# peterdavidfagan/mujoco_robot_environments

Hardware: AMD Instinct MI355X
Metric: env steps/sec (whole node), RearrangementEnv batch=4096 at 1/2/4/8 MI355X (higher is better)
Workload: dtype f32

## Files before the change

### mujoco_robot_environments_amd/csrc/mre_env.h

```cpp
#pragma once
#include <hip/hip_runtime.h>

#include <string>
#include <utility>
#include <vector>

#include "../../include/mre.h"
#include "mre_dev.h"
#include "mre_host.h"
#include "mre_policy.h"

struct mre_env {
  int N = 0, device = 0;
  hipStream_t stream = nullptr;
  mre::DevModel* dM = nullptr;
  mre::DevModel hM;
  int solver = MRE_SOLVER_PGS;
  float *qpos = nullptr, *qvel = nullptr, *qacc_ws = nullptr, *ctrl = nullptr;
  float* qfine = nullptr;
  int *nstep = nullptr, *sv_nstep = nullptr;
  int* nprops = nullptr;
  float* prop_size = nullptr;
  float* osc_target = nullptr;
  uint8_t* grip_closed = nullptr;
// ... 23 lines not shown
  std::vector<std::pair<hipEvent_t, hipEvent_t>> events;
  size_t events_used = 0;
  bool fallback = true;
  unsigned base_flags = 0;
  bool large_only = false;
  bool compact_only = false;
  hipStream_t stream2 = nullptr;
  hipEvent_t ev_fork = nullptr, ev_join = nullptr, ev_order = nullptr;
  uint8_t *d_large = nullptr, *mask_r = nullptr;
  float *sv_qpos = nullptr, *sv_qvel = nullptr, *sv_qacc_ws = nullptr, *sv_ctrl = nullptr, *sv_qfine = nullptr;
  uint32_t* sv_status = nullptr;
  uint8_t* sv_converged = nullptr;
  float* contacts = nullptr;
  float* contacts_full = nullptr;
  int* settle_steps = nullptr;
  int* h_launch_info = nullptr;
  int* d_launch_info = nullptr;
  int* h_info_last = nullptr;
  uint8_t* d_pending = nullptr;
  uint8_t* h_large_stage = nullptr;
  uint8_t* d_large_stage = nullptr;
  bool d_large_stale = false;
  std::vector<uint8_t> h_large, h_rerun;
  int n_large = 0;
  long long* d_env_ids = nullptr;
  int *ps_attempts = nullptr, *ps_prop = nullptr, *ps_tick = nullptr, *ps_which = nullptr;
  double *ps_bounds = nullptr, *ps_pose = nullptr, *ps_zones = nullptr, *ps_pick = nullptr;
  int last_settle_max = 0;
  long long n_reruns = 0, n_promotions = 0, n_demotions = 0;
  struct Group {
    int lo = 0, n = 0;
    hipStream_t st = nullptr, st2 = nullptr;
    hipEvent_t ev_fork = nullptr, ev_join = nullptr;
    struct Out {
      mre::StepArgs args;
      hipEvent_t ev_info = nullptr;
      int stage = 0;
    } out[mre::policy::RING];
    int head = 0, nout = 0;
    int cur = 0;
    int* h_order = nullptr;
    int* d_order = nullptr;
  };
  std::vector<Group> groups;
  int* h_grp_order = nullptr;
  int* d_grp_order = nullptr;
  Group qgroup;
  bool queue_ok = true;
  int queue_ticks = 200;
  int queue_waves = 0;
  int queue_shards = 16;
  int queue_lshards = 8;
  bool queue_test_serial = false;
  int queue_spare_large = 8;
  int queue_run_ticks = 100;
  int queue_min_ticks = 32;
  float tick_tail = 0.f;
  bool tick_tail_valid = false;
  float queue_tail_min = 1.45f;
  unsigned tail_samples = 0;
  std::vector<int> tail_scratch;
  int queue_large_waves_max = 0;
  int* h_qlist = nullptr;
  int* q_ws = nullptr;
  int* q_gen = nullptr;
  int* h_q_err = nullptr;
  int* h_qgrp_order = nullptr;
  long n_queue_launches = 0;
  long long n_handovers = 0;
  int queue_last_handovers = 0;
  static constexpr int RING = mre::policy::RING;
  int ring = 2;
  static constexpr int NSTAGE = mre::policy::NSTAGE;
  hipEvent_t ev_main = nullptr;
  float* seq_copy[RING + 1] = {nullptr, nullptr, nullptr, nullptr, nullptr};
  size_t seq_cap = 0;
  unsigned seq_calls = 0;
  double dbg_wait_s = 0, dbg_call_s = 0; long dbg_calls = 0;
  int calls_since_drain = 0, sync_streak = 0;
  bool broken = false;
};

namespace mre {
int sched_create(mre_env* e);
void sched_destroy(mre_env* e);
int launch_step(mre_env* e, const StepArgs& a, bool settle = false, bool pipeline_ok = true, bool allow_queue = false);
int drain(mre_env* e, bool api_call = false);
}
#define DRAIN(e) do { int rc_ = mre::drain(e, true); if (rc_) return rc_; } while (0)
#define DRAIN_PENDING(e) do { int rc_ = mre::drain(e, false); if (rc_) return rc_; } while (0)

inline int profile_events(mre_env* e, hipEvent_t* e0, hipEvent_t* e1) {
  *e0 = *e1 = nullptr;
  if (!e->profiling) return MRE_OK;
  if (e->events_used == e->events.size()) {
    hipEvent_t x, y;
    HIPCHK(hipEventCreate(&x)); HIPCHK(hipEventCreate(&y));
    e->events.emplace_back(x, y);
  }
  *e0 = e->events[e->events_used].first; *e1 = e->events[e->events_used].second;
  e->events_used++;
  return MRE_OK;
}
```

### mujoco_robot_environments_amd/csrc/mre_kernels.hip

```cpp
#include <hip/hip_runtime.h>

#include "mre_dev.h"
#include "mre_math.h"
#include "mre_collide.h"

namespace mre {
using ModelP = MRE_MODEL_PTR(DevModel);
#if defined(MRE_PHASE_STAMPS) && MRE_PHASE_STAMPS >= 4
__shared__ unsigned long long dbg_acc[4];
#endif

struct OscSm {
  float J[6][7], M[7][7], MiJt[7][6], Li[6][6], Lam[6][6], V[6][6], Jbar[7][6];
  float ep[3], eo[3], F[6], LF[6], tn[7], Jbt[6], xd[6], w[6];
};

struct alignas(8) Blk {
  uint16_t row0;
  uint8_t type, nrows;
  uint8_t rslot;
  uint8_t pa, pb;
  uint8_t primary : 4;
  uint8_t bslot : 4;
};
// ... 1004 lines not shown
      f = (float)(fd - (double)s.qfrc_bias[l]);
    }
    const bool act = prop_is_active(s, dof_pid);
    f = act ? (b < NRB ? f : f - s.qfrc_bias[l]) : 0.f;
    s.qfrc_smooth[l] = f;
    s.qacc_smooth[l] = f;
  }
  MRE_SYNC();
  return arm_mask | (clamped ? 1u << (NU - 1) : 0u);
}
MRE_DEV unsigned smooth_forces(ModelP M, Sm& s, int l) {
  const unsigned arm_mask = arm_actuation(M, s, l);
  const unsigned mask = smooth_forces_assemble(M, s, l, arm_mask);
#ifndef MRE_NEWTON
  solve_robot_one(s.qLD, s.qLDinv, s.qacc_smooth, l);
#else
  factor_solve_robot(s.qM, s.qacc_smooth, l);
#endif
  if (l >= NRV && l < NV) {
    const int p = (l - NRV) / 6, k = (l - NRV) % 6;
    const float md = (k < 3) ? s.prop_mass[p] : s.prop_inertia[p][k - 3];
    s.qacc_smooth[l] = s.qacc_smooth[l] / md;
  }
  MRE_SYNC();
  return mask;
}

MRE_PHASE_FN void integrate_setup(ModelP M, Sm& s, int l, unsigned act_clamped) {
  const bool grip_clamped = (act_clamped >> (NU - 1)) & 1u;
  const float h = M->opt_rec.timestep, grip_bias2 = M->opt_rec.grip_biasprm[2];
  for (int e = l; e < NMR; e += 64) {
    const auto* R = &M->m_rec[e];
    const int i = R->i, j = R->j, ten = R->ten;
    const float damping = R->damping, act_bias2 = R->act_bias2, ten_coef = R->ten_coef;
    float v = s.qM[e];
    if (i == j) {
      v += h * damping;
      if (i < 7 && ((act_clamped >> i) & 1u) == 0u) v -= h * act_bias2;
      if (!grip_clamped) {
        if (ten >= 0) v -= h * grip_bias2 * ten_coef * ten_coef;
      }
    }
    mh_store(s)[e] = v;
#ifdef MRE_NEWTON
    if (i == j) s.scratch[i] = (s.qM[e] - v) * s.qacc[i];
#endif
  }
#ifndef MRE_NEWTON
  if (l < NRV) s.scratch[l] = s.qfrc_smooth[l] + s.qfrc_con[l];
#endif
  MRE_SYNC();
}

MRE_PHASE_FN void integrate(ModelP M, Sm& s, int l, unsigned flags, bool polished, float* clo) {
  const float h = M->opt_rec.timestep;
  const auto* DR = &M->dof_rec[l < NV ? l : 0];
  const int dof_b = DR->body, dof_pid = DR->propid;
  const auto* BR = &M->body_rec[l < NB ? l : 0];
  const int body_qa = BR->qposadr, body_da = BR->dofadr, body_pid = BR->propid;
  const bool freeze = (flags & F_FREEZE_ROBOT) != 0;
  float vl_in = 0.f, ql_in[7] = {0.f, 0.f, 0.f, 0.f, 0.f, 0.f, 0.f};
  if (clo != nullptr) {
    if (l >= NRV && l < NV) vl_in = clo[(QFINE_CUBE_V - QFINE_CUBE_Q) + (l - NRV)];
    if (l >= NRB && l < NB) {
#pragma unroll
      for (int k = 0; k < 7; k++) ql_in[k] = clo[7 * (l - NRB) + k];
    }
  }
  keep_live(dof_pid); keep_live(body_pid); keep_live(body_qa); keep_live(body_da);
  if (l < NV) {
    const int b = dof_b;
    if (b < NRB) {
      if (!freeze) {
#ifdef MRE_NEWTON
        const double acc = polished ? reinterpret_cast<const double*>(&s.nw_Mv[0])[l] : (double)s.qacc[l];
        const double v = robot_v(s, l) + (double)h * (acc + (double)s.scratch[l]);
#else
        const double v = robot_v(s, l) + (double)h * (double)s.scratch[l];
#endif
        const float hi = (float)v;
        s.qvel[l] = hi; s.qlo[QFINE / 2 + l] = (float)(v - (double)hi);
      }
    } else if (prop_is_active(s, dof_pid)) {
      if (clo != nullptr) {
        float* const vl = clo + (QFINE_CUBE_V - QFINE_CUBE_Q) + (l - NRV);
        const double v = (double)s.qvel[l] + (double)vl_in + (double)h * (double)s.qacc[l];
        const float hi = (float)v, lo = (float)(v - (double)hi);
        s.qvel[l] = hi; *vl = lo;
        s.scratch[l] = lo;
      } else {
        s.qvel[l] += h * s.qacc[l];
      }
    }
  }
  MRE_SYNC();
  if (l >= 1 && l < NB) {
    const int b = l, qa = body_qa, da = body_da;
    if (b < NRB) {
      if (!freeze) {
        const double q = robot_q(s, qa) + (double)h * robot_v(s, da);
        const float hi = (float)q;
        s.qpos[qa] = hi; s.qlo[qa] = (float)(q - (double)hi);
      }
    } else if (prop_is_active(s, body_pid) && clo != nullptr) {
      float* const ql = clo + 7 * (b - NRB);
      double vv[6];
      for (int k = 0; k < 6; k++) vv[k] = (double)s.qvel[da + k] + (double)s.scratch[da + k];
      for (int k = 0; k < 3; k++) {
        const double x = (double)s.qpos[qa + k] + (double)ql_in[k] + (double)h * vv[k];
        const float hi = (float)x;
        s.qpos[qa + k] = hi; ql[k] = (float)(x - (double)hi);
      }
      double q0[4], qn[4];
      for (int k = 0; k < 4; k++) q0[k] = (double)s.qpos[qa + 3 + k] + (double)ql_in[3 + k];
      const double wn2 = vv[3] * vv[3] + vv[4] * vv[4] + vv[5] * vv[5];
      if (wn2 > 1e-60) {
        const double inv = rsq64(wn2), half = 0.5 * (double)h * wn2 * inv;
        double sn, cs;
        sincos_poly_d(half, sn, cs);
        const double ax = vv[3] * inv * sn, ay = vv[4] * inv * sn, az = vv[5] * inv * sn;
        qn[0] = q0[0] * cs - q0[1] * ax - q0[2] * ay - q0[3] * az;
        qn[1] = q0[0] * ax + q0[1] * cs + q0[2] * az - q0[3] * ay;
        qn[2] = q0[0] * ay - q0[1] * az + q0[2] * cs + q0[3] * ax;
        qn[3] = q0[0] * az + q0[1] * ay - q0[2] * ax + q0[3] * cs;
      } else {
        for (int k = 0; k < 4; k++) qn[k] = q0[k];
      }
      const double nn = qn[0] * qn[0] + qn[1] * qn[1] + qn[2] * qn[2] + qn[3] * qn[3];
      const double sc = nn > 1e-30 ? rsq64(nn) : 1.0;
      for (int k = 0; k < 4; k++) {
        const double x = qn[k] * sc;
        const float hi = (float)x;
        s.qpos[qa + 3 + k] = hi; ql[3 + k] = (float)(x - (double)hi);
      }
    } else if (prop_is_active(s, body_pid)) {
      for (int k = 0; k < 3; k++) s.qpos[qa + k] += h * s.qvel[da + k];
      float w[3] = {s.qvel[da + 3], s.qvel[da + 4], s.qvel[da + 5]};
      const float ang = v3normalize(w) * h;
      float qr[4], qn[4], q0[4];
      axisangle2q(qr, w, ang);
      for (int k = 0; k < 4; k++) q0[k] = s.qpos[qa + 3 + k];
      qmul(qn, q0, qr);
      qnormalize(qn);
      for (int k = 0; k < 4; k++) s.qpos[qa + 3 + k] = qn[k];
    }
  }
  MRE_SYNC();
}

#ifdef MRE_PHASE_STAMPS
#define MRE_STAMP(k)                                                         \
  do {                                                                       \
    if ((k) < 12 || MRE_PHASE_STAMPS == 3) {                                 \
      const unsigned long long now_ = __builtin_amdgcn_s_memtime();          \
      if ((k) / 4 == MRE_PHASE_STAMPS) stamp_acc[(k) % 4] += now_ - stamp_t; \
      stamp_t = now_;                                                        \
    }                                                                        \
  } while (0)
#else
#define MRE_STAMP(k) do {} while (0)
#endif

MRE_DEV int q_load(const int* p) { return __hip_atomic_load(p, __ATOMIC_RELAXED, __HIP_MEMORY_SCOPE_AGENT); }

#ifdef MRE_LARGE_CAPS
constexpr bool Q_LARGE = true;
#else
constexpr bool Q_LARGE = false;
#endif
MRE_DEV int* q_bucket(const StepArgs& a, int t, int sh) {
  const int S = a.q_shards;
  return a.q_buf + (size_t)t * a.q_stride + (sh < S ? (size_t)sh * a.q_cap : (size_t)S * a.q_cap + (size_t)(sh - S) * a.q_capl);
}

MRE_DEV int queue_pop_shard(const StepArgs& a, int l, int sh, int& env, int& tick) {
  const int S = a.q_shards;
  const bool order0 = sh < S;
  const int n0 = (a.N - sh + S - 1) / S;
  int* const head = a.q_head + sh * QUEUE_TICKS_MAX;
  const int* const tail = a.q_tail + sh * QUEUE_TICKS_MAX;
  for (;;) {
    int h[QUEUE_TICKS_MAX / 64], tl[QUEUE_TICKS_MAX / 64];
#pragma unroll
    for (int c = 0; c < QUEUE_TICKS_MAX / 64; c++) {
      const int b = c * 64 + l;
      h[c] = 0; tl[c] = 0;
      if (b < a.q_nticks) { h[c] = q_load(head + b); tl[c] = (b == 0 && order0) ? n0 : q_load(tail + b); }
    }
    int t = -1, ht = 0;
#pragma unroll
    for (int c = 0; c < QUEUE_TICKS_MAX / 64; c++) {
      if (t < 0 && c * 64 < a.q_nticks) {
        const unsigned long long ready = __ballot(h[c] < tl[c]);
        if (ready != 0ull) {
          const int k = __ffsll((long long)ready) - 1;
          t = c * 64 + k;
          ht = __builtin_amdgcn_readlane(h[c], k);
        }
      }
    }
    if (t < 0) return 0;
    int got = -1;
    if (l == 0) {
      if (t == 0 && order0) {
        const int i = __hip_atomic_fetch_add(head, 1, __ATOMIC_RELAXED, __HIP_MEMORY_SCOPE_AGENT);
        if (i < n0) got = a.env_order != nullptr ? a.env_order[sh + S * i] : sh + S * i;
      } else {
        int expect = ht;
        if (__hip_atomic_compare_exchange_strong(head + t, &expect, ht + 1, __ATOMIC_RELAXED, __ATOMIC_RELAXED,
                                                 __HIP_MEMORY_SCOPE_AGENT)) {
          const int* slot = q_bucket(a, t, sh) + ht;
          int v = q_load(slot);
          for (unsigned spin = 0; v == 0; ++spin) {
            if (spin > (1u << 20)) { *a.q_err = 1; v = -1; break; }
            __builtin_amdgcn_s_sleep(4);
            v = q_load(slot);
          }
          got = v < 0 ? -2 : v - 1;
        }
      }
    }
    got = __builtin_amdgcn_readfirstlane(got);
    if (got == -2) return -1;
    if (got < 0) continue;
    env = got; tick = t;
    return 1;
  }
}
MRE_DEV bool queue_pop(const StepArgs& a, int l, int home, int& env, int& tick, int& shard) {
  const int S = a.q_shards;
  if (Q_LARGE) {
    const int SL = a.q_lshards;
    for (unsigned idle = 0;; ++idle) {
      int r = 0;
      for (int k = 0; k < SL && r == 0; ++k) {
        const int sh = S + (home + k < SL ? home + k : home + k - SL);
        r = queue_pop_shard(a, l, sh, env, tick);
        if (r != 0) shard = sh;
      }
      if (r != 0) return r > 0;
      if (a.q_wait == 0 || q_load(a.q_done) >= a.N) return false;
      if (idle > 512u && q_load(a.q_started) == 0) return false;
      if (idle > (1u << 18)) return false;
      __builtin_amdgcn_s_sleep(127);
    }
  }
  for (int k = 0; k < S; ++k) {
    const int sh = home + k < S ? home + k : home + k - S;
    const int r = queue_pop_shard(a, l, sh, env, tick);
    if (r != 0) { shard = sh; return r > 0; }
  }
  return false;
}
MRE_DEV void queue_push(const StepArgs& a, int l, int env, int tick, int shard) {
  __builtin_amdgcn_fence(__ATOMIC_RELEASE, "agent");
  asm volatile("s_waitcnt vmcnt(0)" ::: "memory");
  if (l == 0) {
    const int i = __hip_atomic_fetch_add(a.q_tail + shard * QUEUE_TICKS_MAX + tick, 1, __ATOMIC_RELAXED, __HIP_MEMORY_SCOPE_AGENT);
    __hip_atomic_store(q_bucket(a, tick, shard) + i, env + 1, __ATOMIC_RELAXED, __HIP_MEMORY_SCOPE_AGENT);
  }
}

template <bool QUEUE>
MRE_DEV void step_body(const StepArgs& a, Sm& s) {
  OscSm& osc = s.osc;
  const int l = threadIdx.x;
  int env = 0, qtick = 0, qshard = 0;
  if (!QUEUE) {
    if ((int)blockIdx.x >= a.N) return;
    env = a.env_order != nullptr ? a.env_order[blockIdx.x] : (int)blockIdx.x;
  }
  if (QUEUE && !Q_LARGE && l == 0) __hip_atomic_fetch_add(a.q_started, 1, __ATOMIC_RELAXED, __HIP_MEMORY_SCOPE_AGENT);
  if (QUEUE && Q_LARGE && a.q_wait != 0) {
    for (unsigned idle = 0; q_load(a.q_gen) != a.q_gen_expect; ++idle) {
      if (idle > 1024u) return;
      __builtin_amdgcn_s_sleep(127);
    }
  }
 for (;;) {
  if (QUEUE) {
    if (!queue_pop(a, l, (int)(blockIdx.x % (unsigned)(Q_LARGE ? a.q_lshards : a.q_shards)), env, qtick, qshard)) return;
    if (qtick > 0 || Q_LARGE) __builtin_amdgcn_fence(__ATOMIC_ACQUIRE, "agent");
  }
  const int step_lo = QUEUE ? qtick * a.control_steps : 0, step_hi = QUEUE ? step_lo + a.control_steps : a.nsteps;
  if (QUEUE && !Q_LARGE && qtick == 0 && a.large != nullptr && a.large[env] != 0) continue;
  if (!QUEUE || (!Q_LARGE && qtick == 0)) {
#define MRE_PASS_SKIP { if (QUEUE) { if (l == 0) __hip_atomic_fetch_add(a.q_done, 1, __ATOMIC_RELAXED, __HIP_MEMORY_SCOPE_AGENT); continue; } return; }
  if (!QUEUE && a.large != nullptr && (a.large[env] != 0) != (a.want_large != 0)) return;
  if (a.env_mask != nullptr && a.env_mask[env] == 0) {
    if (a.launch_info != nullptr && l < 4) a.launch_info[(size_t)env * 4 + l] = -1;
    MRE_PASS_SKIP;
  }
  if (a.pending != nullptr && a.pending[env] != 0) {
    if (a.launch_info != nullptr && l < 4) a.launch_info[(size_t)env * 4 + l] = l == 0 ? -2 : -1;
    MRE_PASS_SKIP;
  }
#undef MRE_PASS_SKIP
  }
  ModelP M = (ModelP)a.M;

  const bool save = a.sv_qpos != nullptr && step_lo == 0;
  if (l < NQP) {
    const float v = a.qpos[(size_t)env * NQP + l];
    s.qpos[l] = v;
    if (save) a.sv_qpos[(size_t)env * NQP + l] = v;
  }
  if (l < NVP) {
    const float v = a.qvel[(size_t)env * NVP + l], w = a.qacc_ws[(size_t)env * NVP + l];
    s.qvel[l] = v;
    s.qacc[l] = w;
    s.qfrc_con[l] = 0.f;
    if (save) { a.sv_qvel[(size_t)env * NVP + l] = v; a.sv_qacc_ws[(size_t)env * NVP + l] = w; }
  }
  if (l < QFINE) {
    const float v = a.qfine != nullptr ? a.qfine[(size_t)env * QFINE_ROW + l] : 0.f;
    s.qlo[l] = v;
    if (save && a.qfine != nullptr) a.sv_qfine[(size_t)env * QFINE_ROW + l] = v;
  }
  if (save && a.qfine != nullptr && l < QFINE_ROW - QFINE)
    a.sv_qfine[(size_t)env * QFINE_ROW + QFINE + l] = a.qfine[(size_t)env * QFINE_ROW + QFINE + l];
  float cube_lo_keep = 0.f;
  if (QUEUE && !Q_LARGE && a.qfine != nullptr && l < QFINE_ROW - QFINE) cube_lo_keep = a.qfine[(size_t)env * QFINE_ROW + QFINE + l];
  if (l < NU) {
    const float v = a.ctrl[(size_t)env * NU + l];
    s.ctrl[l] = v;
    if (save) a.sv_ctrl[(size_t)env * NU + l] = v;
  }
  if (save && l == 0) {
    if (a.nstep != nullptr) a.sv_nstep[env] = a.nstep[env];
    a.sv_status[env] = a.status[env];
    a.sv_converged[env] = a.converged != nullptr ? a.converged[env] : (uint8_t)0;
  }
  if (l == 0) { s.nprops = a.nprops[env]; s.overflow = 0; s.ncon = 0; s.nefc = 0; s.solver_iters = 0; }
#ifdef MRE_NEWTON
  if (l < 24) s.zrow[l] = 0.f;
#endif
  if (l < NPROP * 3) {
    const float sz = a.prop_size[(size_t)env * NPROP * 3 + l];
    s.prop_size[l / 3][l % 3] = sz;
  }
  MRE_SYNC();
  if (l < NPROP) {
    const float m = M->body_mass[NRB + l];
    const float* z = s.prop_size[l];
    s.prop_mass[l] = m;
    s.prop_inertia[l][0] = m / 3.f * (z[1] * z[1] + z[2] * z[2]);
    s.prop_inertia[l][1] = m / 3.f * (z[0] * z[0] + z[2] * z[2]);
    s.prop_inertia[l][2] = m / 3.f * (z[0] * z[0] + z[1] * z[1]);
  }
  MRE_SYNC();

#if defined(MRE_PHASE_STAMPS) && MRE_PHASE_STAMPS >= 4
  if (l < 4) dbg_acc[l] = 0ull;
#endif
#ifdef MRE_PHASE_STAMPS
  unsigned long long stamp_acc[4] = {0, 0, 0, 0};
  unsigned long long stamp_t = __builtin_amdgcn_s_memtime();
#endif
  bool arm_converged = ((a.flags & F_CONV_CONTINUE) != 0 || (QUEUE && qtick > 0)) && a.converged != nullptr && a.converged[env] != 0;
  float grip_cmd = 0.f;
  const OscConfig* oscp = a.osc + (size_t)env * a.osc_stride;
  int hw_ncon = 0, hw_nefc = 0, hw_nrrow = 0, hw_npp = 0;
  const unsigned long long launch_t0 = __builtin_amdgcn_s_memtime();
  if (a.mode == CTRL_OSC) {
    if (l < 16) s.osc_tgt[l] = a.osc_target[(size_t)env * 16 + l];
    grip_cmd = a.grip_closed[env] ? M->act_ctrlrange[NU - 1][1] : M->act_ctrlrange[NU - 1][0];
    MRE_SYNC();
  }
  int steps_done = 0;
  bool settled = false;
  for (int step = step_lo; step < step_hi; ++step) {
    MRE_STAMP(7);
    position_stage(M, s, l);
    MRE_STAMP(12);
    MRE_STAMP(13);
    gripper_local(M, s, l);
    if ((a.flags & F_NO_CONSTRAINTS) == 0) connect_rows_local(M, s, l);
    MRE_STAMP(14);
    crb_mass_matrix(M, s, l);
    MRE_SYNC();
#ifndef MRE_NEWTON
    factor_robot_regs(s.qM, s.qLD, s.qLDinv);
#endif
    MRE_STAMP(15);
    MRE_STAMP(0);

    velocity_stage(M, s, l);
    MRE_SYNC();
    finger_bias(M, s, l);
    MRE_STAMP(1);
    const bool constrained = (a.flags & F_NO_CONSTRAINTS) == 0;
    if (constrained) {

      collide(M, s, l, false, (a.flags & F_CLIP_ALWAYS) != 0);
      MRE_STAMP(2);
      assemble_constraints(M, s, l);
#ifdef MRE_NEWTON
      nw_build_lists(s, l, a.flags);
#else
      solve_robot_rows(s, l);
      assemble_blocks(M, s, l);
#endif
      MRE_STAMP(3);
      hw_ncon = max(hw_ncon, s.ncon); hw_nefc = max(hw_nefc, s.nefc);
      hw_nrrow = max(hw_nrrow, s.nrrow); hw_npp = max(hw_npp, s.npp);
    }

    if (a.mode == CTRL_SEQ && (step % a.control_steps) == 0) {
      const int tick = step / a.control_steps;
      if (l < NU) s.ctrl[l] = a.ctrl_seq[((size_t)tick * a.seq_stride + env) * NU + l];
      MRE_SYNC();
    }
    if (a.mode == CTRL_OSC && (step % a.control_steps) == 0) {
      if (step > 0 && osc_converged(M, s, oscp, s.osc_tgt)) arm_converged = true;
      osc_compute(M, s, osc, oscp, s.osc_tgt, l);
      if (l == 0) s.ctrl[NU - 1] = grip_cmd;
      MRE_SYNC();
    }
    MRE_STAMP(4);
    const unsigned clamped = smooth_forces(M, s, l);
    MRE_STAMP(5);
    bool polished = false;
    if (constrained) {
#if defined(MRE_NEWTON) && defined(MRE_PHASE_STAMPS)
      newton_solve(M, s, l, stamp_acc, stamp_t);
      polished = nw_robot_polish(M, s, l);
#elif defined(MRE_NEWTON)
      newton_solve(M, s, l);
      polished = nw_robot_polish(M, s, l);
#else
      if (M->opt_rec.cone == 0) solve_constraints_pyramidal(M, s, l);
      else solve_constraints(M, s, l);
#endif
      MRE_STAMP(6);
    } else {
      if (l < NVP) { s.qacc[l] = s.qacc_smooth[l]; s.qfrc_con[l] = 0.f; }
      MRE_SYNC();
    }

    integrate_setup(M, s, l, clamped);
    factor_solve_robot(mh_store(s), s.scratch, l);
    integrate(M, s, l, a.flags, polished, a.qfine != nullptr ? a.qfine + (size_t)env * QFINE_ROW + QFINE_CUBE_Q : nullptr);
    steps_done = step + 1 - step_lo;
    if ((a.flags & F_SETTLE_EXIT) != 0) {
      float mv = 0.f, ma = 0.f;
      if (l >= NRV && l < NRV + 6 * s.nprops) { mv = fabsf(s.qvel[l]); ma = fabsf(s.qacc[l]); }
      mv = wave_max(mv); ma = wave_max(ma);
      settled = mv < 1e-3f && ma < 1e-2f && step + 1 > a.min_settle_steps;
    }
    if (a.trace != nullptr && env < a.trace_nenv && (a.trace_base + step) < a.trace_max) {
      if (l < TRACE_QVEL) {
        float v = l < NQ ? s.qpos[l] : 0.f;
        if (l == NQ && constrained) {
          int mask = 0;
          for (int k = 0; k < s.nl; k++) mask |= 1 << ((s.lim_info[k] & 0xFF) - 1);
          v = (float)(s.ncon + 64 * mask);
        }
        if (l == NQ + 1 && constrained) {
          unsigned h = 0u;
          for (int c = 0; c < s.ncon; c++) {
            const int pr = s.con_pair[c];
            const unsigned key = (unsigned)(M->pair_g1[pr] * 32 + M->pair_g2[pr] + 1);
            h = (h + key * key) & 0x3FFFFFu;
          }
          v = (float)h;
        }
        if (l == NQ + 2 && constrained && M->opt_rec.cone != 0) {
          unsigned h = 0u;
          const int ns = 7 + s.nl;
          for (int i = 7; i < ns; i++) h += (s.frc[i] > 0.f ? 1u : 2u) * (unsigned)((i + 1) * (i + 1));
          for (int c = 0; c < s.ncon; c++) {
            const int i = ns + 3 * c;
#ifdef MRE_NEWTON
            const float mu = s.con_fric[c];
#else
            const float mu = s.blkrec[8 + c][15];
#endif
            const float fn = s.frc[i], ft2 = s.frc[i + 1] * s.frc[i + 1] + s.frc[i + 2] * s.frc[i + 2], lim = mu * fn;
            const unsigned z = fn <= 0.f ? 1u : (ft2 >= lim * lim * (1.f - 1e-4f) ? 3u : 2u);
            h += z * (unsigned)((c + 3) * (c + 3));
          }
          v = (float)(h & 0x3FFFFFu);
        }
        a.trace[((size_t)(a.trace_base + step) * a.trace_nenv + env) * TRACE_W + l] = v;
      }
      if (l < NVP) a.trace[((size_t)(a.trace_base + step) * a.trace_nenv + env) * TRACE_W + TRACE_QVEL + l] = l < NV ? s.qvel[l] : 0.f;
    }
    if (settled) break;
  }
  MRE_STAMP(7);
  if (a.settle_steps != nullptr && l == 0) a.settle_steps[env] = settled ? steps_done : -steps_done;
  const bool hand_over = QUEUE && !Q_LARGE && s.overflow != 0;
  if (a.nstep != nullptr && l == 0 && !hand_over) {
    if (QUEUE) __hip_atomic_fetch_add(a.nstep + env, steps_done, __ATOMIC_RELAXED, __HIP_MEMORY_SCOPE_AGENT);
    else a.nstep[env] += steps_done;
  }
  if (a.nsteps == 0 && (a.flags & F_OSC_EVAL) != 0 && a.mode == CTRL_OSC) {
    position_stage(M, s, l);
    gripper_local(M, s, l);
    crb_mass_matrix(M, s, l);
    MRE_SYNC();
    velocity_stage(M, s, l);
    MRE_SYNC();
    osc_compute(M, s, osc, oscp, s.osc_tgt, l);
    if (l == 0) s.ctrl[NU - 1] = grip_cmd;
    MRE_SYNC();
  }
  if (a.nsteps == 0 && (a.flags & F_DETECT) != 0 && a.contacts != nullptr) {
    position_stage(M, s, l);
    collide(M, s, l, (a.flags & F_DETECT_ACTIVE) == 0, (a.flags & F_CLIP_ALWAYS) != 0);
    float* o = a.contacts + (size_t)env * (1 + 3 * CONTACT_EXPORT);
    const int n = s.ncon < CONTACT_EXPORT ? s.ncon : CONTACT_EXPORT;
    if (l == 0) o[0] = s.overflow ? -(float)s.ncon : (float)s.ncon;
    if (l < n) {
      const int pr = s.con_pair[l];
      o[1 + 3 * l] = (float)M->pair_g1[pr]; o[2 + 3 * l] = (float)M->pair_g2[pr]; o[3 + 3 * l] = s.con_dist[l];
      if (a.contacts_full != nullptr) {
        float* f = a.contacts_full + ((size_t)env * CONTACT_EXPORT + l) * 12;
        for (int k = 0; k < 3; k++) f[k] = s.con_pos[l][k];
        for (int k = 0; k < 9; k++) f[3 + k] = s.con_frame[l][k];
      }
    }
    MRE_SYNC();
    if (l == 0) s.overflow = 0;
  }
  const bool q_last = !QUEUE || (qtick + 1 == a.q_nticks && !hand_over);
  if (q_last && (a.mode == CTRL_OSC || a.sites != nullptr || a.geoms != nullptr)) kinematics_only(M, s, l);
  if (a.mode == CTRL_OSC && a.nsteps > 0 && !hand_over) {
    if (q_last && osc_converged(M, s, oscp, s.osc_tgt)) arm_converged = true;
    if (l == 0) {
      if (a.converged != nullptr) a.converged[env] = arm_converged ? 1 : 0;
      if (q_last && !arm_converged && a.status != nullptr && (a.flags & F_CONV_OPEN) == 0) {
        if (QUEUE) __hip_atomic_fetch_or(a.status + env, 1u, __ATOMIC_RELAXED, __HIP_MEMORY_SCOPE_AGENT);
        else a.status[env] |= 1u;
      }
    }
  }
  if (a.geoms != nullptr && l < NG) {
    float p[3], R[9], size[3], rb;
    geom_pose(M, s, l, p, R, size, &rb);
    float* o = a.geoms + ((size_t)env * NG + l) * 16;
    const int pid = M->geom_propid[l];
    const bool active = pid < 0 || pid < s.nprops;
    for (int k = 0; k < 3; k++) o[k] = p[k];
    for (int k = 0; k < 9; k++) o[3 + k] = R[k];
    for (int k = 0; k < 3; k++) o[12 + k] = size[k];
    o[15] = active ? (float)M->geom_type[l] : -1.f;
  }
  if (a.sites != nullptr && q_last) {
    float* o = a.sites + (size_t)env * 16;
    if (l < 3) o[l] = s.site_xpos[M->opt_rec.tcp_site][l];
    if (l >= 3 && l < 6) o[l] = s.site_xpos[M->opt_rec.eef_site][l - 3];
    if (l == 6) {
      float q[4];
      mat2q(q, s.site_xmat[0]);
      o[6] = q[0]; o[7] = q[1]; o[8] = q[2]; o[9] = q[3];
    }
  }
  if (hand_over) {
    if (a.qfine != nullptr && l < QFINE_ROW - QFINE) a.qfine[(size_t)env * QFINE_ROW + QFINE + l] = cube_lo_keep;
  } else {
    if (l < NQP) a.qpos[(size_t)env * NQP + l] = s.qpos[l];
    if (l < NVP) {
      a.qvel[(size_t)env * NVP + l] = s.qvel[l];
      a.qacc_ws[(size_t)env * NVP + l] = l < NV ? s.qacc[l] : 0.f;
    }
    if (l < QFINE && a.qfine != nullptr) a.qfine[(size_t)env * QFINE_ROW + l] = s.qlo[l];
    if (l < NU) a.ctrl[(size_t)env * NU + l] = s.ctrl[l];
  }
  const bool q_more = QUEUE && !hand_over && qtick + 1 < a.q_nticks;
  if (l == 0 && a.launch_info != nullptr) {
    int* li = a.launch_info + (size_t)env * 4;
    unsigned long long dt = (__builtin_amdgcn_s_memtime() - launch_t0) >> 10;
    int moved = 0;
    if (QUEUE) {
      int* qa = a.q_acc + (size_t)env * 4;
      if (qtick > 0 || Q_LARGE) {
        hw_ncon = max(hw_ncon, q_load(qa + 0) & 0xFFFF); hw_nefc = max(hw_nefc, q_load(qa + 1));
        hw_nrrow = max(hw_nrrow, q_load(qa + 2) & 0xFFFF); hw_npp = max(hw_npp, q_load(qa + 2) >> 16);
        dt += (unsigned long long)q_load(qa + 3);
        moved = q_load(qa + 0) >> 16;
      }
      if (hand_over) moved = 1;
      if (q_more || hand_over) { qa[0] = hw_ncon | (moved << 16); qa[1] = hw_nefc; qa[2] = hw_nrrow | (hw_npp << 16); qa[3] = (int)dt; }
      else dt /= (unsigned long long)(qtick + 1);
    }
    if (!q_more && !hand_over) {
#ifdef MRE_LARGE_CAPS
      li[0] = (s.overflow ? 2 : 0) | (moved ? 4 : 0);
#else
      li[0] = s.overflow ? 1 : 0;
#endif
      li[1] = hw_ncon | ((int)(dt < 0x7FFFull ? dt : 0x7FFFull) << 16); li[2] = hw_nefc; li[3] = hw_nrrow | (hw_npp << 16);
    }
  }
#ifndef MRE_LARGE_CAPS
  if (!QUEUE && l == 0 && a.pending != nullptr && s.overflow) a.pending[env] = 1;
#endif
  if (l == 0 && a.status != nullptr && !hand_over) {
    unsigned st = 0;
    for (int k = 0; k < NQ; k++) if (!isfinite(s.qpos[k])) st |= 2u;
    if (s.overflow) st |= 4u;
    if (QUEUE) { if (st) __hip_atomic_fetch_or(a.status + env, st, __ATOMIC_RELAXED, __HIP_MEMORY_SCOPE_AGENT); }
    else a.status[env] |= st;
    if (a.stats != nullptr && a.nsteps > 0) {
      a.stats[env * 4 + 0] = s.ncon; a.stats[env * 4 + 1] = s.nefc;
      a.stats[env * 4 + 2] = s.solver_iters; a.stats[env * 4 + 3] = s.nl;
#ifdef MRE_PHASE_STAMPS
      for (int k = 0; k < 4; k++) a.stats[env * 4 + k] = (int)(stamp_acc[k] >> 4);
#if MRE_PHASE_STAMPS >= 4
      for (int k = 0; k < 4; k++) a.stats[env * 4 + k] = (int)(dbg_acc[k] >> 4);
#endif
#endif
    }
  }
  if (!QUEUE) return;
  if (hand_over) queue_push(a, l, env, qtick, a.q_shards + env % a.q_lshards);
  else if (q_more) queue_push(a, l, env, qtick + 1, qshard);
  else if (l == 0) __hip_atomic_fetch_add(a.q_done, 1, __ATOMIC_RELAXED, __HIP_MEMORY_SCOPE_AGENT);
 }
}

#ifdef MRE_NEWTON
#define MRE_VARIANT(name) name##_newton
#else
#define MRE_VARIANT(name) name
#endif

#ifdef MRE_LARGE_CAPS
__global__ __launch_bounds__(64, 2) void MRE_VARIANT(k_step_large)(StepArgs a) {
  __shared__ Sm s;
  step_body<false>(a, s);
}
}

extern "C" void MRE_VARIANT(mre_launch_step_large)(const mre::StepArgs* args, hipStream_t stream) {
  hipLaunchKernelGGL(mre::MRE_VARIANT(k_step_large), dim3(args->N), dim3(64), 0, stream, *args);
}
namespace mre {
__global__ __launch_bounds__(64, 2) void MRE_VARIANT(k_step_queue_large)(StepArgs a) {
  __shared__ Sm s;
  step_body<true>(a, s);
}
}
extern "C" void MRE_VARIANT(mre_launch_step_queue_large)(const mre::StepArgs* args, int nwaves, hipStream_t stream) {
  hipLaunchKernelGGL(mre::MRE_VARIANT(k_step_queue_large), dim3(nwaves), dim3(64), 0, stream, *args);
}
#else
__global__ __launch_bounds__(64, 2) void MRE_VARIANT(k_step)(StepArgs a) {
  __shared__ Sm s;
  step_body<false>(a, s);
}

__global__ __launch_bounds__(64, 2) void MRE_VARIANT(k_settle)(StepArgs a) {
  __shared__ Sm s;
  step_body<false>(a, s);
}

// ... 360 lines not shown
```

### mujoco_robot_environments_amd/csrc/mre_policy.h

```cpp
#pragma once
#include <algorithm>

#include "mre_dev.h"

namespace mre {
namespace policy {

constexpr int RING = 4;
constexpr int NSTAGE = RING + 1;

inline int info_duration(const int* li) { return li[0] < 0 ? 0 : (li[1] >> 16); }

inline int compact_nrrow_max(bool newton) { return newton ? NRROW_MAX_COMPACT_NEWTON : NRROW_MAX_COMPACT_PGS; }
inline bool near_compact_caps(bool newton, int hw_ncon, int hw_nefc, int hw_nrrow, int hw_npp) {
  return 8 * hw_ncon > 7 * NCON_MAX || 8 * hw_nefc > 7 * NEFC_MAX || 8 * hw_nrrow > 7 * compact_nrrow_max(newton) || 8 * hw_npp > 7 * NPP_MAX;
}
inline bool far_below_compact_caps(bool newton, int hw_ncon, int hw_nefc, int hw_nrrow, int hw_npp) {
  return 8 * hw_ncon <= 5 * NCON_MAX && 8 * hw_nefc <= 5 * NEFC_MAX && 8 * hw_nrrow <= 5 * compact_nrrow_max(newton) && 8 * hw_npp <= 5 * NPP_MAX;
}

enum Action {
  NONE,
  RERUN,
  PROMOTE,
  DEMOTE,
  HANDED_OVER,
};
inline Action decide(const int* li, bool large, bool newton, bool compact_only, bool large_only) {
  if (li[0] < 0) return NONE;
  const int hw_ncon = li[1] & 0xFFFF, hw_nefc = li[2], hw_nrrow = li[3] & 0xFFFF, hw_npp = li[3] >> 16;
  if ((li[0] & 4) != 0 && !large) return HANDED_OVER;
  if (li[0] == 1) return RERUN;
  if (!large) return !compact_only && near_compact_caps(newton, hw_ncon, hw_nefc, hw_nrrow, hw_npp) ? PROMOTE : NONE;
  return !large_only && li[0] == 0 && far_below_compact_caps(newton, hw_ncon, hw_nefc, hw_nrrow, hw_npp) ? DEMOTE : NONE;
}
inline bool flag_after(Action a, bool large) { return a == NONE ? large : a != DEMOTE; }

inline int sort_longest_first(const int* info, int lo, int n, int* order) {
  int kmax = 0;
  for (int i = lo; i < lo + n; i++) kmax = std::max(kmax, info_duration(info + 4 * (size_t)i));
  if (kmax == 0) return 0;
  int count[258] = {0};
  auto bucket = [&](int i) { return (int)((long long)info_duration(info + 4 * (size_t)i) * 255 / kmax); };
  for (int i = lo; i < lo + n; i++) count[255 - bucket(i) + 1]++;
  for (int k = 1; k <= 256; k++) count[k] += count[k - 1];
  for (int i = lo; i < lo + n; i++) order[lo + count[255 - bucket(i)]++] = i;
  return kmax;
}

inline bool tick_tail_ratio(const int* info, int lo, int n, int* scratch, float* ratio) {
  size_t m = 0;
  long long sum = 0;
  for (int i = lo; i < lo + n; i++) {
    const int* li = info + 4 * (size_t)i;
    if (li[0] >= 0) { scratch[m++] = li[1] >> 16; sum += li[1] >> 16; }
  }
  if (m < 256 || sum <= 0) return false;
  const size_t k = m - 1 - m / 100;
  std::nth_element(scratch, scratch + k, scratch + m);
  *ratio = (float)scratch[k] * (float)m / (float)sum;
  return true;
}

inline int free_stage(int cur, const int* younger_stages, int nyounger) {
  bool used[NSTAGE] = {false};
  used[cur] = true;
  for (int k = 0; k < nyounger; k++) used[younger_stages[k]] = true;
  int fs = 0;
  while (used[fs]) fs++;
  return fs;
}

inline int queue_large_waves(const int* info_last, const uint8_t* large, int lo, int n, int nl, int last_handovers,
                             int spare_large, int large_waves_max ) {
  int lw = nl + std::max(last_handovers, spare_large);
  double wl = 0, wc = 0;
  for (int i = lo; i < lo + n; i++) {
    const double d = (double)info_duration(info_last + 4 * (size_t)i);
    if (large[i]) wl += d; else wc += d;
  }
  const double ncomp = (double)(n - nl);
  const double r = (wl > 0 && wc > 0) ? wl / wc : (ncomp > 0 ? 1.3 * (double)nl / ncomp : 1e9);
  const double x = r * 160.0 / (26.5 * r + 20.4);
  const int bal = std::max((int)(x * (double)(large_waves_max / 2)), large_waves_max / 4);
  return std::max(std::min(lw, bal), 1);
}

inline bool queue_fits(bool queue_ok, int queue_waves, int N) { return queue_ok && queue_waves > 0 && N > queue_waves; }
inline bool window_wants_queue(int nticks, int queue_min_ticks, bool tick_tail_valid, float tick_tail, float queue_tail_min) {
  return nticks >= queue_min_ticks || (nticks >= 8 && !(tick_tail_valid && tick_tail < queue_tail_min));
}

inline int ring_keep(int nsteps, int ring) { return nsteps <= 50 ? ring - 1 : 0; }

}
}
```

### mujoco_robot_environments_amd/csrc/mre_sched.cpp

```cpp
#include <hip/hip_runtime.h>
#include <chrono>
#include <cstdlib>
#include <cstring>

#include "mre_env.h"
#include "mre_launch.h"

using namespace mre;

static void launch_compact(const mre_env* e, const StepArgs& a, hipStream_t st, bool settle = false) {
  const StepKernels& K = step_kernels(e->solver);
  (settle ? K.settle : K.step)(&a, st);
}
static void launch_large(const mre_env* e, const StepArgs& a, hipStream_t st) { step_kernels(e->solver).large(&a, st); }

static int launch_split(const mre_env* e, const StepArgs& a, bool run_large, bool settle, hipStream_t st, hipStream_t st2,
                        hipEvent_t ev_fork, hipEvent_t ev_join) {
  StepArgs ac = a;
  ac.want_large = 0;
  if (run_large) {
    HIPCHK(hipEventRecord(ev_fork, st));
    HIPCHK(hipStreamWaitEvent(st2, ev_fork, 0));
    StepArgs al = a;
    al.want_large = 1;
// ... 114 lines not shown
  return drain_group(e, e->qgroup, true);
}

static void guard_args(mre_env* e, StepArgs& a) {
  a.large = e->d_large; a.launch_info = e->d_launch_info;
  a.sv_qpos = e->sv_qpos; a.sv_qvel = e->sv_qvel; a.sv_qacc_ws = e->sv_qacc_ws; a.sv_qfine = e->sv_qfine;
  a.sv_ctrl = e->sv_ctrl; a.sv_status = e->sv_status; a.sv_converged = e->sv_converged; a.sv_nstep = e->sv_nstep;
}

static int launch_group_enqueue(mre_env* e, mre_env::Group& G, const StepArgs& a_full, bool queue) {
  int rc;
  StepArgs a = a_full;
  const size_t N = (size_t)e->N;
  if (G.nout == 0) {
    memcpy(e->h_large_stage + (size_t)G.cur * N + G.lo, e->h_large.data() + G.lo, (size_t)G.n);
    (void)policy::sort_longest_first(e->h_info_last, G.lo, G.n, G.h_order + (size_t)G.cur * N);
  }
  a.N = G.n; a.env_order = G.d_order + (size_t)G.cur * N + G.lo; a.seq_stride = e->N;
  hipEvent_t p0, p1;
  rc = profile_events(e, &p0, &p1);
  if (rc) return rc;
  HIPCHK(hipStreamWaitEvent(G.st, e->ev_main, 0));
  if (p0) HIPCHK(hipEventRecord(p0, G.st));
  guard_args(e, a);
  a.pending = e->d_pending;
  const int slot = (G.head + G.nout) % mre_env::RING;
  a.large = e->d_large_stage + (size_t)G.cur * N;
  a.launch_info = e->d_launch_info + (size_t)slot * 4 * N;
  const uint8_t* const fl = e->h_large_stage + (size_t)G.cur * N;
  if (queue) {
    StepArgs ac = a;
    ac.want_large = 0;
    const StepKernels& K = step_kernels(e->solver);
    const int nt = a.nsteps / a.control_steps, S = e->queue_shards, cap = (G.n + S - 1) / S;
    const int SL = e->queue_lshards, capl = (G.n + SL - 1) / SL;
    constexpr int QS = QUEUE_SHARDS_MAX + QUEUE_LSHARDS_MAX;
    const size_t ctl = 2 * (size_t)QS * QUEUE_TICKS_MAX + 16;
    const size_t stride = (size_t)S * cap + (size_t)SL * capl;
    const size_t words = ctl + 4 * N + (size_t)nt * stride;
    ac.sv_qpos = nullptr;
    ac.q_head = e->q_ws; ac.q_tail = ac.q_head + QS * QUEUE_TICKS_MAX;
    ac.q_done = ac.q_tail + QS * QUEUE_TICKS_MAX; ac.q_started = ac.q_done + 1; ac.q_acc = ac.q_done + 16;
    ac.q_buf = ac.q_acc + 4 * N; ac.q_err = e->h_q_err; ac.q_nticks = nt; ac.q_shards = S; ac.q_cap = cap; ac.q_stride = (int)stride;
    ac.q_lshards = SL; ac.q_capl = capl;
    ac.q_gen = e->q_gen; ac.q_gen_expect = (int)(e->n_queue_launches + 1);
    int* const hl = e->h_qlist + (size_t)(e->n_queue_launches % (mre_env::RING + 1)) * (N + 32);
    int nl = 0;
    for (int j = 0; j < SL; j++) hl[j] = 0;
    memset(hl + 16, 0, (size_t)SL * capl * 4);
    for (int i = G.lo; i < G.lo + G.n; i++)
      if (fl[i]) { const int j = i % SL; hl[16 + (size_t)j * capl + hl[j]++] = i + 1; nl++; }
    StepArgs al = ac;
    al.want_large = 1; al.q_wait = 1;
    const int lw = policy::queue_large_waves(e->h_info_last, fl, G.lo, G.n, nl, e->queue_last_handovers, e->queue_spare_large,
                                             e->queue_large_waves_max);
    hipStream_t const st_large = e->queue_test_serial ? G.st : G.st2;
    K.queue_large(&al, lw, st_large);
    HIPCHK(hipGetLastError());
    HIPCHK(hipEventRecord(G.ev_join, st_large));
    HIPCHK(hipMemsetAsync(e->q_ws, 0, ((words * 4 + 15) / 16) * 16, G.st));
    if (nl > 0) {
      HIPCHK(hipMemcpyAsync(ac.q_buf + (size_t)S * cap, hl + 16, (size_t)SL * capl * 4, hipMemcpyHostToDevice, G.st));
      HIPCHK(hipMemcpy2DAsync(ac.q_tail + S * QUEUE_TICKS_MAX, (size_t)QUEUE_TICKS_MAX * 4, hl, 4, 4, (size_t)SL, hipMemcpyHostToDevice, G.st));
    }
    HIPCHK(hipMemsetD32Async((hipDeviceptr_t)e->q_gen, ac.q_gen_expect, 1, G.st));
    const int nwaves = G.n < e->queue_waves ? G.n : e->queue_waves;
    K.queue(&ac, nwaves, G.st);
    HIPCHK(hipGetLastError());
    al.q_wait = 0;
    const int sweep = G.n < 3 * e->queue_large_waves_max ? G.n : 3 * e->queue_large_waves_max;
    K.queue_large(&al, sweep, G.st);
    e->n_queue_launches++;
    HIPCHK(hipGetLastError());
    HIPCHK(hipStreamWaitEvent(G.st, G.ev_join, 0));
  } else {
    bool run_large = false;
    for (int i = G.lo; i < G.lo + G.n && !run_large; i++) run_large = fl[i] != 0;
    rc = launch_split(e, a, run_large, false, G.st, G.st2, G.ev_fork, G.ev_join);
    if (rc) return rc;
  }
  if (p1) HIPCHK(hipEventRecord(p1, G.st));
  HIPCHK(hipEventRecord(G.out[slot].ev_info, G.st));
  G.out[slot].args = a;
  G.out[slot].stage = G.cur;
  G.nout++;
  return MRE_OK;
}
static int launch_group(mre_env* e, mre_env::Group& G, const StepArgs& a_full, bool queue = false) {
  while (G.nout > policy::ring_keep(a_full.nsteps, e->ring)) {
    int rc = process_oldest(e, G);
    if (rc) return rc;
  }
  int rc = launch_group_enqueue(e, G, a_full, queue);
  if (rc) {
    (void)hipStreamSynchronize(G.st);
    (void)hipStreamSynchronize(G.st2);
    G.nout = 0; G.head = 0;
    (void)hipMemset(e->d_pending + G.lo, 0, (size_t)G.n);
    e->broken = true;
  }
  return rc;
}

int mre::launch_step(mre_env* e, const StepArgs& a, bool settle, bool pipeline_ok, bool allow_queue) {
  if (e->broken) return drain(e);
  HIPCHK(hipSetDevice(e->device));
  const bool guarded = e->fallback && a.nsteps > 0 && (a.flags & F_NO_CONSTRAINTS) == 0;
// ... 172 lines not shown
```

Before: 25.91 million.

## Prefetch next queue item, write-through stores in Newton queue, adaptive spare large waves

```diff
diff --git a/mujoco_robot_environments_amd/csrc/mre_env.h b/mujoco_robot_environments_amd/csrc/mre_env.h
--- a/mujoco_robot_environments_amd/csrc/mre_env.h
+++ b/mujoco_robot_environments_amd/csrc/mre_env.h
@@ -99,7 +99,7 @@
   int queue_shards = 16;
   int queue_lshards = 8;
   bool queue_test_serial = false;
-  int queue_spare_large = 8;
+  int queue_spare_large = -1;
   int queue_run_ticks = 100;
   int queue_min_ticks = 32;
   float tick_tail = 0.f;
diff --git a/mujoco_robot_environments_amd/csrc/mre_kernels.hip b/mujoco_robot_environments_amd/csrc/mre_kernels.hip
--- a/mujoco_robot_environments_amd/csrc/mre_kernels.hip
+++ b/mujoco_robot_environments_amd/csrc/mre_kernels.hip
@@ -1080,6 +1080,26 @@
   MRE_SYNC();
 }
 
+MRE_DEV void q_store(float* p, float v) {
+  __hip_atomic_store(reinterpret_cast<int*>(p), __float_as_int(v), __ATOMIC_RELAXED, __HIP_MEMORY_SCOPE_AGENT);
+}
+MRE_DEV void q_store(int* p, int v) { __hip_atomic_store(p, v, __ATOMIC_RELAXED, __HIP_MEMORY_SCOPE_AGENT); }
+template <bool WT>
+MRE_DEV void travel_store(float* p, float v) {
+  if (WT) q_store(p, v); else *p = v;
+}
+typedef unsigned q_u32x4 __attribute__((ext_vector_type(4)));
+MRE_DEV void q_store_row(float* row, const float* src, int n, int l, bool zero_last = false) {
+  const __amdgpu_buffer_rsrc_t rsrc = __builtin_amdgcn_make_buffer_rsrc(row, 0, n * 4, 0x00020000);
+  if (4 * l < n) {
+    q_u32x4 v;
+    v.x = __float_as_uint(src[4 * l]); v.y = __float_as_uint(src[4 * l + 1]); v.z = __float_as_uint(src[4 * l + 2]);
+    v.w = zero_last && 4 * l + 4 == n ? 0u : __float_as_uint(src[4 * l + 3]);
+    __builtin_amdgcn_raw_buffer_store_b128(v, rsrc, 16 * l, 0, 16 );
+  }
+}
+
+template <bool WT>
 MRE_PHASE_FN void integrate(ModelP M, Sm& s, int l, unsigned flags, bool polished, float* clo) {
   const float h = M->opt_rec.timestep;
   const auto* DR = &M->dof_rec[l < NV ? l : 0];
@@ -1114,7 +1134,7 @@
         float* const vl = clo + (QFINE_CUBE_V - QFINE_CUBE_Q) + (l - NRV);
         const double v = (double)s.qvel[l] + (double)vl_in + (double)h * (double)s.qacc[l];
         const float hi = (float)v, lo = (float)(v - (double)hi);
-        s.qvel[l] = hi; *vl = lo;
+        s.qvel[l] = hi; travel_store<WT>(vl, lo);
         s.scratch[l] = lo;
       } else {
         s.qvel[l] += h * s.qacc[l];
@@ -1137,7 +1157,7 @@
       for (int k = 0; k < 3; k++) {
         const double x = (double)s.qpos[qa + k] + (double)ql_in[k] + (double)h * vv[k];
         const float hi = (float)x;
-        s.qpos[qa + k] = hi; ql[k] = (float)(x - (double)hi);
+        s.qpos[qa + k] = hi; travel_store<WT>(ql + k, (float)(x - (double)hi));
       }
       double q0[4], qn[4];
       for (int k = 0; k < 4; k++) q0[k] = (double)s.qpos[qa + 3 + k] + (double)ql_in[3 + k];
@@ -1159,7 +1179,7 @@
       for (int k = 0; k < 4; k++) {
         const double x = qn[k] * sc;
         const float hi = (float)x;
-        s.qpos[qa + 3 + k] = hi; ql[3 + k] = (float)(x - (double)hi);
+        s.qpos[qa + 3 + k] = hi; travel_store<WT>(ql + 3 + k, (float)(x - (double)hi));
       }
     } else if (prop_is_active(s, body_pid)) {
       for (int k = 0; k < 3; k++) s.qpos[qa + k] += h * s.qvel[da + k];
@@ -1255,7 +1275,7 @@
     return 1;
   }
 }
-MRE_DEV bool queue_pop(const StepArgs& a, int l, int home, int& env, int& tick, int& shard) {
+MRE_DEV bool queue_pop(const StepArgs& a, int l, int home, int& env, int& tick, int& shard, bool wait = true) {
   const int S = a.q_shards;
   if (Q_LARGE) {
     const int SL = a.q_lshards;
@@ -1267,7 +1287,7 @@
         if (r != 0) shard = sh;
       }
       if (r != 0) return r > 0;
-      if (a.q_wait == 0 || q_load(a.q_done) >= a.N) return false;
+      if (!wait || a.q_wait == 0 || q_load(a.q_done) >= a.N) return false;
       if (idle > 512u && q_load(a.q_started) == 0) return false;
       if (idle > (1u << 18)) return false;
       __builtin_amdgcn_s_sleep(127);
@@ -1280,13 +1300,42 @@
   }
   return false;
 }
+#ifdef MRE_NEWTON
+constexpr bool Q_WRITE_THROUGH = true;
+#else
+constexpr bool Q_WRITE_THROUGH = false;
+#endif
 MRE_DEV void queue_push(const StepArgs& a, int l, int env, int tick, int shard) {
-  __builtin_amdgcn_fence(__ATOMIC_RELEASE, "agent");
+  if (!Q_WRITE_THROUGH) __builtin_amdgcn_fence(__ATOMIC_RELEASE, "agent");
   asm volatile("s_waitcnt vmcnt(0)" ::: "memory");
   if (l == 0) {
     const int i = __hip_atomic_fetch_add(a.q_tail + shard * QUEUE_TICKS_MAX + tick, 1, __ATOMIC_RELAXED, __HIP_MEMORY_SCOPE_AGENT);
     __hip_atomic_store(q_bucket(a, tick, shard) + i, env + 1, __ATOMIC_RELAXED, __HIP_MEMORY_SCOPE_AGENT);
   }
+}
+
+struct QueueItem {
+  bool have = false;
+  int env = 0, tick = 0, shard = 0, nprops = 0;
+  float qpos = 0.f, qvel = 0.f, qacc = 0.f, qfine = 0.f, ctrl = 0.f, prop_size = 0.f;
+};
+#ifdef MRE_NEWTON
+constexpr bool Q_EARLY_TAKE = true;
+#else
+constexpr bool Q_EARLY_TAKE = false;
+#endif
+MRE_DEV void queue_take(const StepArgs& a, int l, int home, bool wait, QueueItem& it) {
+  it.have = queue_pop(a, l, home, it.env, it.tick, it.shard, wait);
+  if (!it.have) return;
+  if (it.tick > 0 || Q_LARGE) __builtin_amdgcn_fence(__ATOMIC_ACQUIRE, "agent");
+  const size_t e = (size_t)it.env;
+  it.qpos = l < NQP ? a.qpos[e * NQP + l] : 0.f;
+  it.qvel = l < NVP ? a.qvel[e * NVP + l] : 0.f;
+  it.qacc = l < NVP ? a.qacc_ws[e * NVP + l] : 0.f;
+  it.qfine = l < QFINE && a.qfine != nullptr ? a.qfine[e * QFINE_ROW + l] : 0.f;
+  it.ctrl = l < NU ? a.ctrl[e * NU + l] : 0.f;
+  it.prop_size = l < NPROP * 3 ? a.prop_size[e * NPROP * 3 + l] : 0.f;
+  it.nprops = a.nprops[e];
 }
 
 template <bool QUEUE>
@@ -1305,10 +1354,14 @@
       __builtin_amdgcn_s_sleep(127);
     }
   }
+  const int qhome = QUEUE ? (int)(blockIdx.x % (unsigned)(Q_LARGE ? a.q_lshards : a.q_shards)) : 0;
+  QueueItem next;
  for (;;) {
   if (QUEUE) {
-    if (!queue_pop(a, l, (int)(blockIdx.x % (unsigned)(Q_LARGE ? a.q_lshards : a.q_shards)), env, qtick, qshard)) return;
-    if (qtick > 0 || Q_LARGE) __builtin_amdgcn_fence(__ATOMIC_ACQUIRE, "agent");
+    if (!next.have) queue_take(a, l, qhome, true, next);
+    if (!next.have) return;
+    env = next.env; qtick = next.tick; qshard = next.shard;
+    next.have = false;
   }
   const int step_lo = QUEUE ? qtick * a.control_steps : 0, step_hi = QUEUE ? step_lo + a.control_steps : a.nsteps;
   if (QUEUE && !Q_LARGE && qtick == 0 && a.large != nullptr && a.large[env] != 0) continue;
@@ -1327,21 +1380,21 @@
   }
   ModelP M = (ModelP)a.M;
 
-  const bool save = a.sv_qpos != nullptr && step_lo == 0;
+  const bool save = !QUEUE && a.sv_qpos != nullptr && step_lo == 0;
   if (l < NQP) {
-    const float v = a.qpos[(size_t)env * NQP + l];
+    const float v = QUEUE ? next.qpos : a.qpos[(size_t)env * NQP + l];
     s.qpos[l] = v;
     if (save) a.sv_qpos[(size_t)env * NQP + l] = v;
   }
   if (l < NVP) {
-    const float v = a.qvel[(size_t)env * NVP + l], w = a.qacc_ws[(size_t)env * NVP + l];
+    const float v = QUEUE ? next.qvel : a.qvel[(size_t)env * NVP + l], w = QUEUE ? next.qacc : a.qacc_ws[(size_t)env * NVP + l];
     s.qvel[l] = v;
     s.qacc[l] = w;
     s.qfrc_con[l] = 0.f;
     if (save) { a.sv_qvel[(size_t)env * NVP + l] = v; a.sv_qacc_ws[(size_t)env * NVP + l] = w; }
   }
   if (l < QFINE) {
-    const float v = a.qfine != nullptr ? a.qfine[(size_t)env * QFINE_ROW + l] : 0.f;
+    const float v = QUEUE ? next.qfine : a.qfine != nullptr ? a.qfine[(size_t)env * QFINE_ROW + l] : 0.f;
     s.qlo[l] = v;
     if (save && a.qfine != nullptr) a.sv_qfine[(size_t)env * QFINE_ROW + l] = v;
   }
@@ -1350,7 +1403,7 @@
   float cube_lo_keep = 0.f;
   if (QUEUE && !Q_LARGE && a.qfine != nullptr && l < QFINE_ROW - QFINE) cube_lo_keep = a.qfine[(size_t)env * QFINE_ROW + QFINE + l];
   if (l < NU) {
-    const float v = a.ctrl[(size_t)env * NU + l];
+    const float v = QUEUE ? next.ctrl : a.ctrl[(size_t)env * NU + l];
     s.ctrl[l] = v;
     if (save) a.sv_ctrl[(size_t)env * NU + l] = v;
   }
@@ -1359,12 +1412,12 @@
     a.sv_status[env] = a.status[env];
     a.sv_converged[env] = a.converged != nullptr ? a.converged[env] : (uint8_t)0;
   }
-  if (l == 0) { s.nprops = a.nprops[env]; s.overflow = 0; s.ncon = 0; s.nefc = 0; s.solver_iters = 0; }
+  if (l == 0) { s.nprops = QUEUE ? next.nprops : a.nprops[env]; s.overflow = 0; s.ncon = 0; s.nefc = 0; s.solver_iters = 0; }
 #ifdef MRE_NEWTON
   if (l < 24) s.zrow[l] = 0.f;
 #endif
   if (l < NPROP * 3) {
-    const float sz = a.prop_size[(size_t)env * NPROP * 3 + l];
+    const float sz = QUEUE ? next.prop_size : a.prop_size[(size_t)env * NPROP * 3 + l];
     s.prop_size[l / 3][l % 3] = sz;
   }
   MRE_SYNC();
@@ -1466,9 +1519,13 @@
       MRE_SYNC();
     }
 
+    if (QUEUE && Q_EARLY_TAKE && step + 1 == step_hi) queue_take(a, l, qhome, false, next);
+    float cube_lo_warm = 0.f;
+    if (QUEUE && Q_WRITE_THROUGH && a.qfine != nullptr && l < QFINE_ROW - QFINE) cube_lo_warm = a.qfine[(size_t)env * QFINE_ROW + QFINE + l];
     integrate_setup(M, s, l, clamped);
     factor_solve_robot(mh_store(s), s.scratch, l);
-    integrate(M, s, l, a.flags, polished, a.qfine != nullptr ? a.qfine + (size_t)env * QFINE_ROW + QFINE_CUBE_Q : nullptr);
+    if (QUEUE && Q_WRITE_THROUGH) keep_live(cube_lo_warm);
+    integrate<QUEUE && Q_WRITE_THROUGH>(M, s, l, a.flags, polished, a.qfine != nullptr ? a.qfine + (size_t)env * QFINE_ROW + QFINE_CUBE_Q : nullptr);
     steps_done = step + 1 - step_lo;
     if ((a.flags & F_SETTLE_EXIT) != 0) {
       float mv = 0.f, ma = 0.f;
@@ -1510,15 +1567,28 @@
           }
           v = (float)(h & 0x3FFFFFu);
         }
-        a.trace[((size_t)(a.trace_base + step) * a.trace_nenv + env) * TRACE_W + l] = v;
+        travel_store<QUEUE && Q_WRITE_THROUGH>(&a.trace[((size_t)(a.trace_base + step) * a.trace_nenv + env) * TRACE_W + l], v);
       }
-      if (l < NVP) a.trace[((size_t)(a.trace_base + step) * a.trace_nenv + env) * TRACE_W + TRACE_QVEL + l] = l < NV ? s.qvel[l] : 0.f;
+      if (l < NVP)
+        travel_store<QUEUE && Q_WRITE_THROUGH>(&a.trace[((size_t)(a.trace_base + step) * a.trace_nenv + env) * TRACE_W + TRACE_QVEL + l],
+                                               l < NV ? s.qvel[l] : 0.f);
     }
     if (settled) break;
   }
   MRE_STAMP(7);
   if (a.settle_steps != nullptr && l == 0) a.settle_steps[env] = settled ? steps_done : -steps_done;
   const bool hand_over = QUEUE && !Q_LARGE && s.overflow != 0;
+  if (QUEUE && Q_WRITE_THROUGH) {
+    if (hand_over) {
+      if (a.qfine != nullptr && l < QFINE_ROW - QFINE) q_store(a.qfine + (size_t)env * QFINE_ROW + QFINE + l, cube_lo_keep);
+    } else {
+      q_store_row(a.qpos + (size_t)env * NQP, s.qpos, NQP, l);
+      q_store_row(a.qvel + (size_t)env * NVP, s.qvel, NVP, l);
+      q_store_row(a.qacc_ws + (size_t)env * NVP, s.qacc, NVP, l, true);
+      if (a.qfine != nullptr) q_store_row(a.qfine + (size_t)env * QFINE_ROW, s.qlo, QFINE, l);
+      q_store_row(a.ctrl + (size_t)env * NU, s.ctrl, NU, l);
+    }
+  }
   if (a.nstep != nullptr && l == 0 && !hand_over) {
     if (QUEUE) __hip_atomic_fetch_add(a.nstep + env, steps_done, __ATOMIC_RELAXED, __HIP_MEMORY_SCOPE_AGENT);
     else a.nstep[env] += steps_done;
@@ -1557,7 +1627,10 @@
   if (a.mode == CTRL_OSC && a.nsteps > 0 && !hand_over) {
     if (q_last && osc_converged(M, s, oscp, s.osc_tgt)) arm_converged = true;
     if (l == 0) {
-      if (a.converged != nullptr) a.converged[env] = arm_converged ? 1 : 0;
+      if (a.converged != nullptr) {
+        if (QUEUE && Q_WRITE_THROUGH) __hip_atomic_store(a.converged + env, (uint8_t)(arm_converged ? 1 : 0), __ATOMIC_RELAXED, __HIP_MEMORY_SCOPE_AGENT);
+        else a.converged[env] = arm_converged ? 1 : 0;
+      }
       if (q_last && !arm_converged && a.status != nullptr && (a.flags & F_CONV_OPEN) == 0) {
         if (QUEUE) __hip_atomic_fetch_or(a.status + env, 1u, __ATOMIC_RELAXED, __HIP_MEMORY_SCOPE_AGENT);
         else a.status[env] |= 1u;
@@ -1585,7 +1658,8 @@
       o[6] = q[0]; o[7] = q[1]; o[8] = q[2]; o[9] = q[3];
     }
   }
-  if (hand_over) {
+  if (QUEUE && Q_WRITE_THROUGH) {
+  } else if (hand_over) {
     if (a.qfine != nullptr && l < QFINE_ROW - QFINE) a.qfine[(size_t)env * QFINE_ROW + QFINE + l] = cube_lo_keep;
   } else {
     if (l < NQP) a.qpos[(size_t)env * NQP + l] = s.qpos[l];
@@ -1610,7 +1684,11 @@
         moved = q_load(qa + 0) >> 16;
       }
       if (hand_over) moved = 1;
-      if (q_more || hand_over) { qa[0] = hw_ncon | (moved << 16); qa[1] = hw_nefc; qa[2] = hw_nrrow | (hw_npp << 16); qa[3] = (int)dt; }
+      if ((q_more || hand_over) && Q_WRITE_THROUGH) {
+        q_store(qa + 0, hw_ncon | (moved << 16)); q_store(qa + 1, hw_nefc); q_store(qa + 2, hw_nrrow | (hw_npp << 16)); q_store(qa + 3, (int)dt);
+      } else if (q_more || hand_over) {
+        qa[0] = hw_ncon | (moved << 16); qa[1] = hw_nefc; qa[2] = hw_nrrow | (hw_npp << 16); qa[3] = (int)dt;
+      }
       else dt /= (unsigned long long)(qtick + 1);
     }
     if (!q_more && !hand_over) {
@@ -1631,7 +1709,7 @@
     if (s.overflow) st |= 4u;
     if (QUEUE) { if (st) __hip_atomic_fetch_or(a.status + env, st, __ATOMIC_RELAXED, __HIP_MEMORY_SCOPE_AGENT); }
     else a.status[env] |= st;
-    if (a.stats != nullptr && a.nsteps > 0) {
+    if (a.stats != nullptr && a.nsteps > 0 && !(QUEUE && Q_WRITE_THROUGH && q_more)) {
       a.stats[env * 4 + 0] = s.ncon; a.stats[env * 4 + 1] = s.nefc;
       a.stats[env * 4 + 2] = s.solver_iters; a.stats[env * 4 + 3] = s.nl;
 #ifdef MRE_PHASE_STAMPS
diff --git a/mujoco_robot_environments_amd/csrc/mre_policy.h b/mujoco_robot_environments_amd/csrc/mre_policy.h
--- a/mujoco_robot_environments_amd/csrc/mre_policy.h
+++ b/mujoco_robot_environments_amd/csrc/mre_policy.h
@@ -71,6 +71,12 @@
   return fs;
 }
 
+constexpr int QUEUE_SPARE_LARGE_QUIET = 1, QUEUE_SPARE_LARGE_BUSY = 8;
+inline int queue_spare_large(int last_handovers, int forced) {
+  if (forced >= 0) return forced;
+  return last_handovers > 0 ? QUEUE_SPARE_LARGE_BUSY : QUEUE_SPARE_LARGE_QUIET;
+}
+
 inline int queue_large_waves(const int* info_last, const uint8_t* large, int lo, int n, int nl, int last_handovers,
                              int spare_large, int large_waves_max ) {
   int lw = nl + std::max(last_handovers, spare_large);
diff --git a/mujoco_robot_environments_amd/csrc/mre_sched.cpp b/mujoco_robot_environments_amd/csrc/mre_sched.cpp
--- a/mujoco_robot_environments_amd/csrc/mre_sched.cpp
+++ b/mujoco_robot_environments_amd/csrc/mre_sched.cpp
@@ -190,7 +190,8 @@
       if (fl[i]) { const int j = i % SL; hl[16 + (size_t)j * capl + hl[j]++] = i + 1; nl++; }
     StepArgs al = ac;
     al.want_large = 1; al.q_wait = 1;
-    const int lw = policy::queue_large_waves(e->h_info_last, fl, G.lo, G.n, nl, e->queue_last_handovers, e->queue_spare_large,
+    const int lw = policy::queue_large_waves(e->h_info_last, fl, G.lo, G.n, nl, e->queue_last_handovers,
+                                             policy::queue_spare_large(e->queue_last_handovers, e->queue_spare_large),
                                              e->queue_large_waves_max);
     hipStream_t const st_large = e->queue_test_serial ? G.st : G.st2;
     K.queue_large(&al, lw, st_large);
```

After: 26.55 million, median of 6. 1.02x the previous value.
